# NVlabs/FoundationPose

Hardware: NVIDIA H100
Metric: pose-hypotheses/sec at 640x480 RGB-D, 252 hyp, 5 refine iters (higher is better)
Workload: dtype f16

## Files before the change

foundationpose_b200/csrc/fp_gemm.cu:

```cuda
#include "fp_gemm.cuh"

#include <stdarg.h>
#include <stdlib.h>
#include <string.h>

#include <mutex>
#include <vector>

#include "fp_common.cuh"
#include "fp_wgmma.cuh"

namespace fp {

static std::atomic<unsigned long long> g_launch_count{0};
static thread_local bool t_capturing = false;
void note_launches(int n) {
  if (!t_capturing) g_launch_count.fetch_add((unsigned long long)n, std::memory_order_relaxed);
}
unsigned long long launch_count() { return g_launch_count.load(std::memory_order_relaxed); }
void set_capturing(bool on) { t_capturing = on; }

std::atomic<bool> g_prof_on{false};
static std::mutex g_prof_mu;

struct ProfRec {
  cudaEvent_t e0, e1;
  double work;
  int kind;
};
static std::vector<ProfRec> g_prof_recs;

void prof_mark_begin(int kind, double work, cudaStream_t stream) {
  if (!g_prof_on) return;
  ProfRec r;
  r.kind = kind;
  r.work = work;
  cudaEventCreate(&r.e0);
  cudaEventCreate(&r.e1);
  cudaEventRecord(r.e0, stream);
  std::lock_guard<std::mutex> lk(g_prof_mu);
  g_prof_recs.push_back(r);
}
void prof_mark_end(cudaStream_t stream) {
  if (!g_prof_on) return;
  std::lock_guard<std::mutex> lk(g_prof_mu);
  if (g_prof_recs.empty()) return;
  cudaEventRecord(g_prof_recs.back().e1, stream);
}
int prof_collect(int kind, double* total_ms, double* total_work, int* launches) {
  FP_CUDA_OK(cudaDeviceSynchronize());
  std::lock_guard<std::mutex> lk(g_prof_mu);
  double ms = 0, work = 0;
  int n = 0;
  std::vector<ProfRec> keep;
  for (auto& r : g_prof_recs) {
    if (r.kind != kind) {
      keep.push_back(r);
      continue;
    }
    float t = 0.f;
    cudaEventElapsedTime(&t, r.e0, r.e1);
    ms += t;
    work += r.work;
    ++n;
    cudaEventDestroy(r.e0);
    cudaEventDestroy(r.e1);
  }
  g_prof_recs.swap(keep);
  *total_ms = ms;
  *total_work = work;
  *launches = n;
  return 0;
}

static thread_local char t_last_error[1024] = "";
void set_last_error(const char* fmt, ...) {
  va_list ap;
  va_start(ap, fmt);
  vsnprintf(t_last_error, sizeof(t_last_error), fmt, ap);
  va_end(ap);
}
const char* get_last_error() { return t_last_error; }

static thread_local int t_pdl_skip = 0;
void pdl_skip_next() { t_pdl_skip = 1; }

bool pdl_enabled() {
  if (t_pdl_skip) {
    t_pdl_skip = 0;
    return false;
  }
  static int on = -1;
  if (on < 0) {
    const char* e = getenv("FPOSE_PDL");
    on = (e && e[0] == '0') ? 0 : 1;
  }
  return on != 0;
}

struct GemmParams {
  int lg_bw, lg_bh;
  int bw, bh, bn;
  int tiles_w, tiles_h, tiles_n, n_tiles_n, total_tiles;
  int num_kb, chunks_per_tap;
  int dim_w, dim_h, dim_n;
  short tap_off[9][5];
  int Ho, Wo, n_img, Cout;
  const float* bias;
  int has_res;
  int odim_h, odim_n;
  int out_split;
  const float* post_add;
  int relu;
  double alg_flops;
};

constexpr int kBlockM = 128;
constexpr int kBlockK = 64;
constexpr int kABytes = kBlockM * kBlockK * 2;
constexpr int kTileThreads = 384;
constexpr int kSlabBytes = kBlockM * 64 * 2;
constexpr int kSmemOptIn = 232448;

constexpr int kWideSlabs = 2;
constexpr int kWideProducerRegs = 40;
constexpr int kWideConsumerRegs = 232;
template <int BN>
struct TileCfg {
  static constexpr int kBBytes = BN * kBlockK * 2;
  static constexpr int kStageBytes = kABytes + kBBytes;
  static constexpr int kBatches = BN / 64;
  static constexpr bool kAlternate = BN > 128;
  static constexpr int kSlabs = kAlternate ? kWideSlabs : kBatches;
  static constexpr int kStagingBytes = kSlabs * kSlabBytes;
  static constexpr int kRing = kSmemOptIn - kStagingBytes - 1024  - 256 ;
  static constexpr int kStages = (kRing / kStageBytes) > 8 ? 8 : (kRing / kStageBytes);
  static constexpr int kSmemBytes = kStages * kStageBytes + kStagingBytes + 1024 + 256;
  static_assert(kSmemBytes <= kSmemOptIn, "tile configuration exceeds the 227 KB opt-in shared memory");
  static_assert((2 * kStages + kSlabs) * 8 <= 256, "the mbarriers must fit their 256 bytes");
  static_assert(kBatches % kSlabs == 0, "every slab must take the same number of batches per tile");
};

template <int BN>
__global__ void __launch_bounds__(kTileThreads, 1)
    gemm_tile_kernel(const __grid_constant__ CUtensorMap map_a, const __grid_constant__ CUtensorMap map_b,
                     const __grid_constant__ CUtensorMap map_out, const __grid_constant__ CUtensorMap map_res,
                     const __grid_constant__ GemmParams p) {
  using Cfg = TileCfg<BN>;
  constexpr int S = Cfg::kStages;
  constexpr int NSLAB = Cfg::kSlabs;
  constexpr int NB = Cfg::kBatches;
  constexpr bool kAlt = Cfg::kAlternate;
  extern __shared__ uint8_t smem_raw[];
  uint8_t* smem = smem_raw + ((1024u - (smem_u32(smem_raw) & 1023u)) & 1023u);
  uint8_t* staging = smem + S * Cfg::kStageBytes;
  uint64_t* bars = reinterpret_cast<uint64_t*>(staging + Cfg::kStagingBytes);
  uint64_t* full = bars;
  uint64_t* empty = bars + S;
  uint64_t* res_full = bars + 2 * S;

  const int m_tiles = p.tiles_w * p.tiles_h * p.tiles_n;
  const int total = m_tiles * p.n_tiles_n;

  if (threadIdx.x == 0) {
    tma_prefetch_desc(&map_a);
    tma_prefetch_desc(&map_b);
    tma_prefetch_desc(&map_out);
    if (p.has_res) tma_prefetch_desc(&map_res);
    for (int s = 0; s < S; ++s) {
      mbar_init(&full[s], 1);
      mbar_init(&empty[s], 256);
    }
    for (int s = 0; s < (kAlt ? NSLAB : 1); ++s) mbar_init(&res_full[s], 1);
    mbar_fence_init();
  }
  __syncthreads();
  pdl_trigger();
  pdl_wait();

  auto decode = [&](int t, int& n_tile, int& tw, int& th, int& tn) {
    n_tile = t % p.n_tiles_n;
    const int m_tile = t / p.n_tiles_n;
    tw = m_tile % p.tiles_w;
    th = (m_tile / p.tiles_w) % p.tiles_h;
    tn = m_tile / (p.tiles_w * p.tiles_h);
  };

  if (threadIdx.x < 128) {
    if constexpr (BN > 128) regs_release<kWideProducerRegs>();
    if (threadIdx.x == 0) {
      int stage = 0, phase = 0;
      for (int t = blockIdx.x; t < total; t += gridDim.x) {
        int n_tile, tw, th, tn;
        decode(t, n_tile, tw, th, tn);
        int base[5] = {0, 0, 0, 0, 0};
        base[p.dim_w] += tw * p.bw;
        if (p.dim_h >= 0) base[p.dim_h] += th * p.bh;
        if (p.dim_n >= 0) base[p.dim_n] += tn * p.bn;
        int tap = 0, chunk = 0;
        for (int kb = 0; kb < p.num_kb; ++kb) {
          mbar_wait(&empty[stage], phase ^ 1);
          uint8_t* sa = smem + stage * Cfg::kStageBytes;
          mbar_expect_tx(&full[stage], Cfg::kStageBytes);
          tma_load_5d(&map_a, &full[stage], sa, base[0] + p.tap_off[tap][0] + chunk * kBlockK, base[1] + p.tap_off[tap][1],
                      base[2] + p.tap_off[tap][2], base[3] + p.tap_off[tap][3], base[4] + p.tap_off[tap][4]);
          tma_load_2d(&map_b, &full[stage], sa + kABytes, kb * kBlockK, n_tile * BN);
          if (++chunk == p.chunks_per_tap) {
            chunk = 0;
            ++tap;
          }
          if (++stage == S) {
            stage = 0;
            phase ^= 1;
          }
        }
      }
    }
    return;
  }

  if constexpr (BN > 128) regs_acquire<kWideConsumerRegs>();
  const int ct = threadIdx.x - 128;
  const int cw = ct >> 7;
  const int lane = threadIdx.x & 31;
  const int r0 = 64 * cw + 16 * ((ct >> 5) & 3) + (lane >> 2);
  const int cq = 2 * (lane & 3);
  const bool leader = (ct == 0);
  float acc[BN / 2];
#pragma unroll
  for (int i = 0; i < BN / 2; ++i) acc[i] = 0.f;
  int stage = 0, phase = 0, it = 0;
  for (int t = blockIdx.x; t < total; t += gridDim.x, ++it) {
    int n_tile, tw, th, tn;
    decode(t, n_tile, tw, th, tn);
    const int n0 = tn * p.bn;
    int n_o0 = n0, coff = 0;
    if (p.out_split > 0) {
      n_o0 = n0 % p.out_split;
      coff = (n0 / p.out_split) * p.Cout;
    }
    int oc[5] = {0, 0, 0, 0, 0}, rc[5] = {0, 0, 0, 0, 0};
    oc[1] = rc[1] = tw * p.bw;
    if (p.odim_h >= 0) oc[p.odim_h] = rc[p.odim_h] = th * p.bh;
    if (p.odim_n >= 0) {
      oc[p.odim_n] = n_o0;
      rc[p.odim_n] = n0;
    }
    if (leader) asm volatile("cp.async.bulk.wait_group.read 0;" ::: "memory");
    asm volatile("bar.sync 1, 256;" ::: "memory");
    if (leader && p.has_res) {
      for (int s = 0; s < NSLAB; ++s) {
        uint64_t* rb = &res_full[kAlt ? s : 0];
        if (kAlt || s == 0) mbar_expect_tx(rb, kAlt ? kSlabBytes : NSLAB * kSlabBytes);
        tma_load_5d(&map_res, rb, staging + s * kSlabBytes, n_tile * BN + s * 64, rc[1], rc[2], rc[3], rc[4]);
      }
    }

    int prev = -1;
    for (int kb = 0; kb < p.num_kb; ++kb) {
      mbar_wait(&full[stage], phase);
      const uint32_t sa = smem_u32(smem + stage * Cfg::kStageBytes);
      const uint64_t da = gmma_desc_sw128(sa + (uint32_t)cw * 8192u);
      const uint64_t db = gmma_desc_sw128(sa + kABytes);
      wgmma_fence();
#pragma unroll
      for (int k = 0; k < kBlockK / 16; ++k)
        Wgmma<BN>::ss(acc, da + (uint64_t)(2 * k), db + (uint64_t)(2 * k), (kb > 0 || k > 0) ? 1u : 0u);
      wgmma_commit();
      if (prev >= 0) {
        wgmma_wait<1>();
        mbar_arrive(&empty[prev]);
      }
      prev = stage;
      if (++stage == S) {
        stage = 0;
        phase ^= 1;
      }
    }
    const float* bias = p.bias + n_tile * BN;
    const float* pap[2] = {nullptr, nullptr};
    if (p.post_add) {
#pragma unroll
      for (int h = 0; h < 2; ++h) {
        const int row = r0 + 8 * h;
        const int jj = row & (p.bw - 1), ii = (row >> p.lg_bw) & (p.bh - 1);
        const int i = th * p.bh + ii, j = min(tw * p.bw + jj, p.Wo - 1);
        pap[h] = p.post_add + (size_t)(i * p.Wo + j) * p.Cout + n_tile * BN;
      }
    }
    float2 pe[8][2];
    auto load_pe = [&](int b) {
#pragma unroll
      for (int jl = 0; jl < 8; ++jl)
#pragma unroll
        for (int h = 0; h < 2; ++h) pe[jl][h] = __ldg(reinterpret_cast<const float2*>(pap[h] + 64 * b + 8 * jl + cq));
    };
    if (p.post_add) load_pe(0);
    wgmma_wait<0>();
    fence_regs(acc);
    if (prev >= 0) mbar_arrive(&empty[prev]);

#pragma unroll
    for (int b = 0; b < NB; ++b) {
      const int s = kAlt ? (b & 1) : b;
      uint8_t* slab = staging + s * kSlabBytes;
      if (kAlt && p.has_res && b > 0 && b + 1 < NB) {
        if (leader) {
          asm volatile("cp.async.bulk.wait_group.read 0;" ::: "memory");
          uint64_t* rb = &res_full[(b + 1) & 1];
          mbar_expect_tx(rb, kSlabBytes);
          tma_load_5d(&map_res, rb, staging + ((b + 1) & 1) * kSlabBytes, n_tile * BN + (b + 1) * 64, rc[1], rc[2],
                      rc[3], rc[4]);
        }
      }
      if (p.has_res && (kAlt || b == 0))
        mbar_wait(&res_full[kAlt ? s : 0], (uint32_t)((it * (NB / NSLAB) + b / NSLAB) & 1));
#pragma unroll
      for (int jh = 0; jh < 8; jh += 4) {
        float2 bb[4];
        __half2 rv[4][2];
#pragma unroll
        for (int jl = 0; jl < 4; ++jl) {
          bb[jl] = __ldg(reinterpret_cast<const float2*>(bias + 64 * b + 8 * (jh + jl) + cq));
          if (p.has_res) {
#pragma unroll
            for (int h = 0; h < 2; ++h) {
              const int row = r0 + 8 * h;
              rv[jl][h] = *reinterpret_cast<const __half2*>(slab + row * 128 + (((uint32_t)(jh + jl) ^ (uint32_t)(row & 7)) << 4) + cq * 2);
            }
          }
        }
#pragma unroll
        for (int jl = 0; jl < 4; ++jl) {
          const int j = 8 * b + jh + jl;
#pragma unroll
          for (int h = 0; h < 2; ++h) {
            const int row = r0 + 8 * h;
            uint32_t* cell = reinterpret_cast<uint32_t*>(slab + row * 128 + (((uint32_t)(jh + jl) ^ (uint32_t)(row & 7)) << 4) + cq * 2);
            float a0 = acc[4 * j + 2 * h] + bb[jl].x, a1 = acc[4 * j + 2 * h + 1] + bb[jl].y;
            if (p.has_res) {
              const float2 r = __half22float2(rv[jl][h]);
              a0 += r.x;
              a1 += r.y;
            }
            if (p.relu) {
              a0 = fmaxf(a0, 0.f);
              a1 = fmaxf(a1, 0.f);
            }
            if (p.post_add) {
              a0 += pe[jh + jl][h].x;
              a1 += pe[jh + jl][h].y;
            }
            *cell = pack_half2(a0, a1);
          }
        }
      }
      if (p.post_add && b + 1 < NB) load_pe(b + 1);
      if (kAlt || b == NB - 1) {
        asm volatile("fence.proxy.async.shared::cta;" ::: "memory");
        if (kAlt && leader) asm volatile("cp.async.bulk.wait_group.read 0;" ::: "memory");
        asm volatile("bar.sync 1, 256;" ::: "memory");
        if (leader) {
          for (int q = kAlt ? s : 0; q < (kAlt ? s + 1 : NSLAB); ++q)
            tma_store_5d(&map_out, staging + q * kSlabBytes, coff + n_tile * BN + (kAlt ? 64 * b : 64 * q), oc[1],
                         oc[2], oc[3], oc[4]);
          asm volatile("cp.async.bulk.commit_group;" ::: "memory");
        }
      }
    }
  }
  if (leader) asm volatile("cp.async.bulk.wait_group 0;" ::: "memory");
}

static int g_num_sms = 0;

typedef CUresult (*EncodeTiledFn)(CUtensorMap*, CUtensorMapDataType, cuuint32_t, void*, const cuuint64_t*,
                                  const cuuint64_t*, const cuuint32_t*, const cuuint32_t*,
                                  CUtensorMapInterleave, CUtensorMapSwizzle, CUtensorMapL2promotion,
                                  CUtensorMapFloatOOBfill);

static EncodeTiledFn get_encode_fn() {
  static EncodeTiledFn fn = nullptr;
  static std::once_flag once;
  std::call_once(once, [] {
    void* p = nullptr;
    cudaDriverEntryPointQueryResult qres;
    if (cudaGetDriverEntryPoint("cuTensorMapEncodeTiled", &p, cudaEnableDefault, &qres) == cudaSuccess &&
        qres == cudaDriverEntryPointSuccess)
      fn = reinterpret_cast<EncodeTiledFn>(p);
  });
  return fn;
}

static int encode_map(CUtensorMap* map, const void* base, int rank, const uint64_t* dims,
                      const uint64_t* strides_bytes , const uint32_t* box, bool swizzle128 = true) {
  EncodeTiledFn fn = get_encode_fn();
  FP_REQUIRE(fn != nullptr, "cuTensorMapEncodeTiled entry point not available (no CUDA driver?)");
  cuuint64_t gdim[5];
  cuuint64_t gstr[4];
  cuuint32_t bdim[5];
  cuuint32_t estr[5];
  for (int i = 0; i < rank; ++i) {
    gdim[i] = dims[i];
    bdim[i] = box[i];
    estr[i] = 1;
  }
  for (int i = 0; i < rank - 1; ++i) gstr[i] = strides_bytes[i];
  CUresult r = fn(map, CU_TENSOR_MAP_DATA_TYPE_FLOAT16, (cuuint32_t)rank, const_cast<void*>(base), gdim, gstr,
                  bdim, estr, CU_TENSOR_MAP_INTERLEAVE_NONE, swizzle128 ? CU_TENSOR_MAP_SWIZZLE_128B : CU_TENSOR_MAP_SWIZZLE_NONE,
                  CU_TENSOR_MAP_L2_PROMOTION_L2_256B, CU_TENSOR_MAP_FLOAT_OOB_FILL_NONE);
  FP_REQUIRE(r == CUDA_SUCCESS,
             "cuTensorMapEncodeTiled failed (%d): rank %d dims [%llu %llu %llu %llu %llu] box [%u %u %u %u %u]",
             (int)r, rank, (unsigned long long)dims[0], (unsigned long long)(rank > 1 ? dims[1] : 0),
             (unsigned long long)(rank > 2 ? dims[2] : 0), (unsigned long long)(rank > 3 ? dims[3] : 0),
             (unsigned long long)(rank > 4 ? dims[4] : 0), box[0], rank > 1 ? box[1] : 0, rank > 2 ? box[2] : 0,
             rank > 3 ? box[3] : 0, rank > 4 ? box[4] : 0);
  return 0;
}

int encode_map_f16(CUtensorMap* map, const void* base, int rank, const uint64_t* dims, const uint64_t* strides_bytes,
                   const uint32_t* box) {
  return encode_map(map, base, rank, dims, strides_bytes, box);
}
int encode_map_f16_linear(CUtensorMap* map, const void* base, int rank, const uint64_t* dims,
                          const uint64_t* strides_bytes, const uint32_t* box) {
  return encode_map(map, base, rank, dims, strides_bytes, box, false);
}
int num_sms() {
  if (g_num_sms == 0) {
    int dev = 0;
    if (cudaGetDevice(&dev) != cudaSuccess) return 0;
    if (cudaDeviceGetAttribute(&g_num_sms, cudaDevAttrMultiProcessorCount, dev) != cudaSuccess) return 0;
  }
  return g_num_sms;
}

static int ilog2(int v) {
  int l = 0;
  while ((1 << l) < v) ++l;
  return l;
}

template <int BN>
static int launch_bn(const CUtensorMap& ma, const CUtensorMap& mb, const CUtensorMap& mo, const CUtensorMap& mr,
                     const GemmParams& p, cudaStream_t stream) {
  using Cfg = TileCfg<BN>;
  static std::atomic<unsigned long long> attr_mask{0};
  if (!device_bit_test(attr_mask)) {
    FP_CUDA_OK(cudaFuncSetAttribute(gemm_tile_kernel<BN>, cudaFuncAttributeMaxDynamicSharedMemorySize, Cfg::kSmemBytes));
    device_bit_set(attr_mask);
  }
  const int sms = num_sms();
  FP_REQUIRE(sms > 0, "no CUDA device");
  const int grid = p.total_tiles < sms ? p.total_tiles : sms;
  prof_mark_begin(0, p.alg_flops, stream);
  FP_CUDA_OK(launch_pdl(gemm_tile_kernel<BN>, dim3(grid), dim3(kTileThreads), Cfg::kSmemBytes, stream, 1, ma, mb, mo, mr, p));
  prof_mark_end(stream);
  note_launches(1);
  FP_CUDA_OK(cudaGetLastError());
  return 0;
}

int stem_conv_launch(const GemmLayer& L, cudaStream_t stream);

static int gemm_layer_plan(const GemmLayer& L, cudaStream_t stream, int* tile_n) {
  if (L.kind == LK_CONV7_S2) {
    if (tile_n) {
      *tile_n = 64;
      return 0;
    }
    return stem_conv_launch(L, stream);
  }
  GemmParams p;
  memset(&p, 0, sizeof(p));
  CUtensorMap ma, mb;
  const uint64_t E = 2;
  int Ho, Wo, taps, ktot;
  int BN;
  uint64_t dims[5], str[4];
  uint32_t box[5];

  switch (L.kind) {
    case LK_LINEAR: {
      FP_REQUIRE(L.Cin % 64 == 0, "LINEAR: K=%d not a multiple of 64", L.Cin);
      Ho = 1;
      Wo = L.Win;
      taps = 1;
      p.chunks_per_tap = L.Cin / 64;
      p.bw = 128; p.bh = 1; p.bn = 1;
      p.dim_w = 1; p.dim_h = -1; p.dim_n = -1;
      dims[0] = L.Cin; dims[1] = L.Win; dims[2] = 1; dims[3] = 1; dims[4] = 1;
      str[0] = L.Cin * E; str[1] = str[0] * L.Win; str[2] = str[1]; str[3] = str[1];
      box[0] = 64; box[1] = 128; box[2] = 1; box[3] = 1; box[4] = 1;
      p.tiles_w = (L.Win + 127) / 128; p.tiles_h = 1; p.tiles_n = 1;
      break;
    }
    case LK_CONV3_S1: {
      FP_REQUIRE(L.Cin % 64 == 0, "CONV3_S1: Cin=%d not a multiple of 64", L.Cin);
      Ho = L.Hin; Wo = L.Win;
      taps = 9;
      p.chunks_per_tap = L.Cin / 64;
      if (Wo % 8 == 0 && Ho % 8 == 0) { p.bw = 8; p.bh = 8; p.bn = 2; }
      else if (Wo % 4 == 0 && Ho % 4 == 0) { p.bw = 4; p.bh = 4; p.bn = 8; }
      else FP_REQUIRE(false, "CONV3_S1: unsupported spatial size %dx%d", Ho, Wo);
      const uint64_t sw_ = (uint64_t)L.Cin * E, sh_ = sw_ * L.Win, sn_ = sh_ * L.Hin;
      p.dim_w = 1; p.dim_h = 2; p.dim_n = 3;
      dims[0] = L.Cin; dims[1] = L.Win; dims[2] = L.Hin; dims[3] = L.n_img; dims[4] = 1;
      str[0] = sw_; str[1] = sh_; str[2] = sn_; str[3] = sn_ * L.n_img;
      box[0] = 64; box[1] = p.bw; box[2] = p.bh; box[3] = p.bn; box[4] = 1;
      for (int r = 0; r < 3; ++r)
        for (int s = 0; s < 3; ++s) {
          p.tap_off[r * 3 + s][1] = (short)(s - 1);
          p.tap_off[r * 3 + s][2] = (short)(r - 1);
        }
      p.tiles_w = Wo / p.bw; p.tiles_h = Ho / p.bh; p.tiles_n = (L.n_img + p.bn - 1) / p.bn;
      break;
    }
    case LK_CONV3_S2: {
      FP_REQUIRE(L.Cin % 64 == 0, "CONV3_S2: Cin=%d not a multiple of 64", L.Cin);
      FP_REQUIRE(L.Hin % 2 == 0 && L.Win % 2 == 0, "CONV3_S2: odd input size");
      Ho = L.Hin / 2; Wo = L.Win / 2;
      taps = 9;
      p.chunks_per_tap = L.Cin / 64;
      if (Wo % 8 == 0 && Ho % 8 == 0) { p.bw = 8; p.bh = 8; p.bn = 2; }
      else if (Wo % 4 == 0 && Ho % 4 == 0) { p.bw = 4; p.bh = 4; p.bn = 8; }
      else FP_REQUIRE(false, "CONV3_S2: unsupported output size %dx%d", Ho, Wo);
      p.dim_w = 1; p.dim_h = 3; p.dim_n = 4;
      dims[0] = 2 * L.Cin; dims[1] = Wo; dims[2] = 2; dims[3] = Ho; dims[4] = L.n_img;
      str[0] = 2 * L.Cin * E; str[1] = (uint64_t)L.Win * L.Cin * E; str[2] = 2 * str[1];
      str[3] = (uint64_t)L.Hin * L.Win * L.Cin * E;
      box[0] = 64; box[1] = p.bw; box[2] = 1; box[3] = p.bh; box[4] = p.bn;
      for (int r = 0; r < 3; ++r)
        for (int s = 0; s < 3; ++s) {
          const int t = r * 3 + s;
          p.tap_off[t][0] = (short)((s == 1 ? 0 : 1) * L.Cin);
          p.tap_off[t][1] = (short)(s == 0 ? -1 : 0);
          p.tap_off[t][2] = (short)(r == 1 ? 0 : 1);
          p.tap_off[t][3] = (short)(r == 0 ? -1 : 0);
        }
      p.tiles_w = Wo / p.bw; p.tiles_h = Ho / p.bh; p.tiles_n = (L.n_img + p.bn - 1) / p.bn;
      break;
    }
    default:
      FP_REQUIRE(false, "unknown layer kind %d", L.kind);
  }
  ktot = taps * L.Cin;
  p.num_kb = ktot / 64;
  p.lg_bw = ilog2(p.bw);
  p.lg_bh = ilog2(p.bh);

  constexpr int kWideMinWaves = 8;
  constexpr int kWideMinKBlocks = 16;
  const int m_tiles = p.tiles_w * p.tiles_h * p.tiles_n;
  if (L.Cout % 256 == 0 && p.num_kb >= kWideMinKBlocks) {
    const int sms = num_sms();
    FP_REQUIRE(sms > 0, "no CUDA device");
    BN = (long long)m_tiles * (L.Cout / 256) >= (long long)kWideMinWaves * sms ? 256 : 128;
  } else if (L.Cout % 128 == 0) BN = 128;
  else if (L.Cout % 64 == 0) BN = 64;
  else FP_REQUIRE(false, "Cout=%d must be a multiple of 64", L.Cout);
  p.n_tiles_n = L.Cout / BN;
  p.total_tiles = p.tiles_w * p.tiles_h * p.tiles_n * p.n_tiles_n;
  p.Ho = Ho; p.Wo = Wo; p.n_img = L.n_img; p.Cout = L.Cout;
  p.bias = L.bias;
  p.has_res = L.res != nullptr;
  p.out_split = L.out_split;
  p.post_add = L.post_add;
  p.relu = L.relu;
  {
    const double k_real = (double)taps * L.Cin;
    p.alg_flops = 2.0 * (double)L.n_img * Ho * Wo * L.Cout * k_real;
  }
  FP_REQUIRE(L.out_ld % 8 == 0 && (!L.res || L.res_ld % 8 == 0), "out_ld / res_ld must be multiples of 8");
  FP_REQUIRE(L.out_split == 0 || L.out_split % p.bn == 0,
             "out_split=%d must be a multiple of the tile's image count %d (pad the A/B batch boundary)", L.out_split,
             p.bn);
  if (tile_n) {
    *tile_n = BN;
    return 0;
  }
  if (p.total_tiles == 0) return 0;

  int rc = encode_map(&ma, L.in, 5, dims, str, box);
  if (rc) return rc;
  uint64_t wd[2] = {(uint64_t)ktot, (uint64_t)L.Cout};
  uint64_t ws[1] = {(uint64_t)ktot * E};
  uint32_t wb[2] = {64, (uint32_t)BN};
  rc = encode_map(&mb, L.w, 2, wd, ws, wb);
  if (rc) return rc;
  CUtensorMap mo, mr;
  {
    uint64_t od[5], os[4];
    uint32_t ob[5];
    const bool lin = (L.kind == LK_LINEAR);
    const int n_out = L.out_split > 0 ? (L.n_img - L.out_split) : L.n_img;
    FP_REQUIRE(n_out > 0, "out_split=%d leaves no output images (n_img=%d)", L.out_split, L.n_img);
    auto fill = [&](int ld, int nimg) {
      const uint64_t sw_ = (uint64_t)ld * E, sh_ = sw_ * Wo, sn_ = sh_ * Ho;
      od[0] = (uint64_t)ld;
      ob[0] = 64;
      od[4] = 1;
      ob[4] = 1;
      if (lin) {
        od[1] = (uint64_t)Wo; od[2] = 1; od[3] = 1;
        os[0] = sw_; os[1] = sh_; os[2] = sh_; os[3] = sh_;
        ob[1] = (uint32_t)p.bw; ob[2] = 1; ob[3] = 1;
      } else {
        od[1] = (uint64_t)Wo; od[2] = (uint64_t)Ho; od[3] = (uint64_t)nimg;
        os[0] = sw_; os[1] = sh_; os[2] = sn_; os[3] = sn_ * nimg;
        ob[1] = (uint32_t)p.bw; ob[2] = (uint32_t)p.bh; ob[3] = (uint32_t)p.bn;
      }
    };
    p.odim_h = lin ? -1 : 2;
    p.odim_n = lin ? -1 : 3;
    fill(L.out_ld, n_out);
    rc = encode_map(&mo, L.out, 5, od, os, ob);
    if (rc) return rc;
    if (L.res) {
      fill(L.res_ld, L.n_img);
      rc = encode_map(&mr, L.res, 5, od, os, ob);
      if (rc) return rc;
    } else {
      mr = mo;
    }
  }
  if (BN == 256) return launch_bn<256>(ma, mb, mo, mr, p, stream);
  return BN == 128 ? launch_bn<128>(ma, mb, mo, mr, p, stream) : launch_bn<64>(ma, mb, mo, mr, p, stream);
}

int gemm_layer_launch(const GemmLayer& L, cudaStream_t stream) { return gemm_layer_plan(L, stream, nullptr); }

int gemm_layer_tile_n(const GemmLayer& L, int* tile_n) { return gemm_layer_plan(L, nullptr, tile_n); }

}
```

Before: 3611.

## Overlap next tile's first k-blocks with epilogue using double accumulators

```diff
diff --git a/foundationpose_b200/csrc/fp_gemm.cu b/foundationpose_b200/csrc/fp_gemm.cu
--- a/foundationpose_b200/csrc/fp_gemm.cu
+++ b/foundationpose_b200/csrc/fp_gemm.cu
@@ -123,8 +123,10 @@
 constexpr int kSmemOptIn = 232448;
 
 constexpr int kWideSlabs = 2;
-constexpr int kWideProducerRegs = 40;
-constexpr int kWideConsumerRegs = 232;
+constexpr int kProducerRegs = 40;
+constexpr int kConsumerRegs = 232;
+constexpr int kOverlapHead = 3;
+constexpr int kOverlapMaxKBlocks = 8;
 template <int BN>
 struct TileCfg {
   static constexpr int kBBytes = BN * kBlockK * 2;
@@ -139,7 +141,53 @@
   static_assert(kSmemBytes <= kSmemOptIn, "tile configuration exceeds the 227 KB opt-in shared memory");
   static_assert((2 * kStages + kSlabs) * 8 <= 256, "the mbarriers must fit their 256 bytes");
   static_assert(kBatches % kSlabs == 0, "every slab must take the same number of batches per tile");
+  static_assert(kAlternate || kOverlapHead < kStages, "the overlapped k-blocks need free ring stages");
 };
+
+template <int BN>
+__device__ __forceinline__ void convert_batch(const float (&acc)[BN / 2], int b, uint8_t* slab, const float* bias,
+                                              const float2 (&pe)[8][2], const GemmParams& p, int r0, int cq) {
+#pragma unroll
+  for (int jh = 0; jh < 8; jh += 4) {
+    float2 bb[4];
+    __half2 rv[4][2];
+#pragma unroll
+    for (int jl = 0; jl < 4; ++jl) {
+      bb[jl] = __ldg(reinterpret_cast<const float2*>(bias + 64 * b + 8 * (jh + jl) + cq));
+      if (p.has_res) {
+#pragma unroll
+        for (int h = 0; h < 2; ++h) {
+          const int row = r0 + 8 * h;
+          rv[jl][h] = *reinterpret_cast<const __half2*>(slab + row * 128 + (((uint32_t)(jh + jl) ^ (uint32_t)(row & 7)) << 4) + cq * 2);
+        }
+      }
+    }
+#pragma unroll
+    for (int jl = 0; jl < 4; ++jl) {
+      const int j = 8 * b + jh + jl;
+#pragma unroll
+      for (int h = 0; h < 2; ++h) {
+        const int row = r0 + 8 * h;
+        uint32_t* cell = reinterpret_cast<uint32_t*>(slab + row * 128 + (((uint32_t)(jh + jl) ^ (uint32_t)(row & 7)) << 4) + cq * 2);
+        float a0 = acc[4 * j + 2 * h] + bb[jl].x, a1 = acc[4 * j + 2 * h + 1] + bb[jl].y;
+        if (p.has_res) {
+          const float2 r = __half22float2(rv[jl][h]);
+          a0 += r.x;
+          a1 += r.y;
+        }
+        if (p.relu) {
+          a0 = fmaxf(a0, 0.f);
+          a1 = fmaxf(a1, 0.f);
+        }
+        if (p.post_add) {
+          a0 += pe[jh + jl][h].x;
+          a1 += pe[jh + jl][h].y;
+        }
+        *cell = pack_half2(a0, a1);
+      }
+    }
+  }
+}
 
 template <int BN>
 __global__ void __launch_bounds__(kTileThreads, 1)
@@ -187,7 +235,7 @@
   };
 
   if (threadIdx.x < 128) {
-    if constexpr (BN > 128) regs_release<kWideProducerRegs>();
+    regs_release<kProducerRegs>();
     if (threadIdx.x == 0) {
       int stage = 0, phase = 0;
       for (int t = blockIdx.x; t < total; t += gridDim.x) {
@@ -219,45 +267,53 @@
     return;
   }
 
-  if constexpr (BN > 128) regs_acquire<kWideConsumerRegs>();
+  regs_acquire<kConsumerRegs>();
   const int ct = threadIdx.x - 128;
   const int cw = ct >> 7;
   const int lane = threadIdx.x & 31;
   const int r0 = 64 * cw + 16 * ((ct >> 5) & 3) + (lane >> 2);
   const int cq = 2 * (lane & 3);
   const bool leader = (ct == 0);
-  float acc[BN / 2];
-#pragma unroll
-  for (int i = 0; i < BN / 2; ++i) acc[i] = 0.f;
-  int stage = 0, phase = 0, it = 0;
-  for (int t = blockIdx.x; t < total; t += gridDim.x, ++it) {
-    int n_tile, tw, th, tn;
-    decode(t, n_tile, tw, th, tn);
-    const int n0 = tn * p.bn;
-    int n_o0 = n0, coff = 0;
-    if (p.out_split > 0) {
-      n_o0 = n0 % p.out_split;
-      coff = (n0 / p.out_split) * p.Cout;
-    }
-    int oc[5] = {0, 0, 0, 0, 0}, rc[5] = {0, 0, 0, 0, 0};
-    oc[1] = rc[1] = tw * p.bw;
-    if (p.odim_h >= 0) oc[p.odim_h] = rc[p.odim_h] = th * p.bh;
-    if (p.odim_n >= 0) {
-      oc[p.odim_n] = n_o0;
-      rc[p.odim_n] = n0;
-    }
-    if (leader) asm volatile("cp.async.bulk.wait_group.read 0;" ::: "memory");
-    asm volatile("bar.sync 1, 256;" ::: "memory");
-    if (leader && p.has_res) {
-      for (int s = 0; s < NSLAB; ++s) {
-        uint64_t* rb = &res_full[kAlt ? s : 0];
-        if (kAlt || s == 0) mbar_expect_tx(rb, kAlt ? kSlabBytes : NSLAB * kSlabBytes);
-        tma_load_5d(&map_res, rb, staging + s * kSlabBytes, n_tile * BN + s * 64, rc[1], rc[2], rc[3], rc[4]);
-      }
-    }
-
-    int prev = -1;
-    for (int kb = 0; kb < p.num_kb; ++kb) {
+  if constexpr (!kAlt) {
+    int stage = 0, phase = 0;
+
+    auto tile_coords = [&](int t, int& n_tile, int& tw, int& th, int& coff, int (&oc)[5], int (&rc)[5]) {
+      int tn;
+      decode(t, n_tile, tw, th, tn);
+      const int n0 = tn * p.bn;
+      int n_o0 = n0;
+      coff = 0;
+      if (p.out_split > 0) {
+        n_o0 = n0 % p.out_split;
+        coff = (n0 / p.out_split) * p.Cout;
+      }
+#pragma unroll
+      for (int d = 0; d < 5; ++d) oc[d] = rc[d] = 0;
+      oc[1] = rc[1] = tw * p.bw;
+      if (p.odim_h >= 0) oc[p.odim_h] = rc[p.odim_h] = th * p.bh;
+      if (p.odim_n >= 0) {
+        oc[p.odim_n] = n_o0;
+        rc[p.odim_n] = n0;
+      }
+    };
+    const float* pap[2] = {nullptr, nullptr};
+    float2 pe[8][2];
+    auto pe_rows = [&](int n_tile, int tw, int th) {
+#pragma unroll
+      for (int h = 0; h < 2; ++h) {
+        const int row = r0 + 8 * h;
+        const int jj = row & (p.bw - 1), ii = (row >> p.lg_bw) & (p.bh - 1);
+        const int i = th * p.bh + ii, j = min(tw * p.bw + jj, p.Wo - 1);
+        pap[h] = p.post_add + (size_t)(i * p.Wo + j) * p.Cout + n_tile * BN;
+      }
+    };
+    auto load_pe = [&](int b) {
+#pragma unroll
+      for (int jl = 0; jl < 8; ++jl)
+#pragma unroll
+        for (int h = 0; h < 2; ++h) pe[jl][h] = __ldg(reinterpret_cast<const float2*>(pap[h] + 64 * b + 8 * jl + cq));
+    };
+    auto mma_kblock = [&](float (&acc)[BN / 2], int kb) {
       mbar_wait(&full[stage], phase);
       const uint32_t sa = smem_u32(smem + stage * Cfg::kStageBytes);
       const uint64_t da = gmma_desc_sw128(sa + (uint32_t)cw * 8192u);
@@ -267,104 +323,233 @@
       for (int k = 0; k < kBlockK / 16; ++k)
         Wgmma<BN>::ss(acc, da + (uint64_t)(2 * k), db + (uint64_t)(2 * k), (kb > 0 || k > 0) ? 1u : 0u);
       wgmma_commit();
-      if (prev >= 0) {
-        wgmma_wait<1>();
-        mbar_arrive(&empty[prev]);
-      }
-      prev = stage;
       if (++stage == S) {
         stage = 0;
         phase ^= 1;
       }
-    }
-    const float* bias = p.bias + n_tile * BN;
-    const float* pap[2] = {nullptr, nullptr};
-    if (p.post_add) {
-#pragma unroll
-      for (int h = 0; h < 2; ++h) {
-        const int row = r0 + 8 * h;
-        const int jj = row & (p.bw - 1), ii = (row >> p.lg_bw) & (p.bh - 1);
-        const int i = th * p.bh + ii, j = min(tw * p.bw + jj, p.Wo - 1);
-        pap[h] = p.post_add + (size_t)(i * p.Wo + j) * p.Cout + n_tile * BN;
-      }
-    }
-    float2 pe[8][2];
-    auto load_pe = [&](int b) {
-#pragma unroll
-      for (int jl = 0; jl < 8; ++jl)
-#pragma unroll
-        for (int h = 0; h < 2; ++h) pe[jl][h] = __ldg(reinterpret_cast<const float2*>(pap[h] + 64 * b + 8 * jl + cq));
     };
-    if (p.post_add) load_pe(0);
-    wgmma_wait<0>();
-    fence_regs(acc);
-    if (prev >= 0) mbar_arrive(&empty[prev]);
-
-#pragma unroll
-    for (int b = 0; b < NB; ++b) {
-      const int s = kAlt ? (b & 1) : b;
-      uint8_t* slab = staging + s * kSlabBytes;
-      if (kAlt && p.has_res && b > 0 && b + 1 < NB) {
-        if (leader) {
-          asm volatile("cp.async.bulk.wait_group.read 0;" ::: "memory");
-          uint64_t* rb = &res_full[(b + 1) & 1];
-          mbar_expect_tx(rb, kSlabBytes);
-          tma_load_5d(&map_res, rb, staging + ((b + 1) & 1) * kSlabBytes, n_tile * BN + (b + 1) * 64, rc[1], rc[2],
-                      rc[3], rc[4]);
-        }
-      }
-      if (p.has_res && (kAlt || b == 0))
-        mbar_wait(&res_full[kAlt ? s : 0], (uint32_t)((it * (NB / NSLAB) + b / NSLAB) & 1));
-#pragma unroll
-      for (int jh = 0; jh < 8; jh += 4) {
-        float2 bb[4];
-        __half2 rv[4][2];
-#pragma unroll
-        for (int jl = 0; jl < 4; ++jl) {
-          bb[jl] = __ldg(reinterpret_cast<const float2*>(bias + 64 * b + 8 * (jh + jl) + cq));
-          if (p.has_res) {
+
+    float acc0[BN / 2], acc1[BN / 2];
+    const int head = min(kOverlapHead, p.num_kb);
+    int rel = 0, held = 0;
+    auto release_to = [&](int keep) {
+      for (; held > keep; --held) {
+        mbar_arrive(&empty[rel]);
+        if (++rel == S) rel = 0;
+      }
+    };
+    int issued = 0;
+    auto run_tile = [&](float (&acc)[BN / 2], float (&nxt)[BN / 2], int t, int it) {
+      int n_tile, tw, th, coff, oc[5], rc[5];
+      tile_coords(t, n_tile, tw, th, coff, oc, rc);
+      if (leader && p.has_res) {
+        asm volatile("cp.async.bulk.wait_group.read 0;" ::: "memory");
+        mbar_expect_tx(&res_full[0], NSLAB * kSlabBytes);
+        for (int s = 0; s < NSLAB; ++s)
+          tma_load_5d(&map_res, &res_full[0], staging + s * kSlabBytes, n_tile * BN + s * 64, rc[1], rc[2], rc[3], rc[4]);
+      }
+      for (int kb = issued; kb < p.num_kb; ++kb) {
+        mma_kblock(acc, kb);
+        ++held;
+        wgmma_wait<1>();
+        release_to(1);
+      }
+      const float* bias = p.bias + n_tile * BN;
+      if (p.post_add) {
+        pe_rows(n_tile, tw, th);
+        load_pe(0);
+      }
+      const bool has_next = t + (int)gridDim.x < total;
+      const bool overlap = has_next && head == kOverlapHead && p.num_kb <= kOverlapMaxKBlocks;
+      issued = 0;
+      if (overlap) {
+        wgmma_wait<0>();
+        release_to(0);
+#pragma unroll
+        for (int kb = 0; kb < kOverlapHead; ++kb) mma_kblock(nxt, kb);
+        issued = kOverlapHead;
+        held += kOverlapHead;
+      } else {
+        if (has_next)
+          for (; issued < head; ++issued) mma_kblock(nxt, issued);
+        held += issued;
+        wgmma_wait<0>();
+        release_to(0);
+      }
+      fence_regs(acc);
+      if (p.has_res) {
+        mbar_wait(&res_full[0], (uint32_t)(it & 1));
+      } else {
+        if (leader) asm volatile("cp.async.bulk.wait_group.read 0;" ::: "memory");
+        asm volatile("bar.sync 1, 256;" ::: "memory");
+      }
+#pragma unroll
+      for (int b = 0; b < NB; ++b) {
+        convert_batch<BN>(acc, b, staging + b * kSlabBytes, bias, pe, p, r0, cq);
+        if (b + 1 < NB) {
+          if (p.post_add) load_pe(b + 1);
+          if (overlap && issued < p.num_kb) {
+            mma_kblock(nxt, issued++);
+            ++held;
+            wgmma_wait<kOverlapHead>();
+            release_to(kOverlapHead);
+          }
+        }
+      }
+      asm volatile("fence.proxy.async.shared::cta;" ::: "memory");
+      asm volatile("bar.sync 1, 256;" ::: "memory");
+      if (leader) {
+        for (int q = 0; q < NSLAB; ++q)
+          tma_store_5d(&map_out, staging + q * kSlabBytes, coff + n_tile * BN + 64 * q, oc[1], oc[2], oc[3], oc[4]);
+        asm volatile("cp.async.bulk.commit_group;" ::: "memory");
+      }
+    };
+    for (int t = blockIdx.x, it = 0; t < total; t += gridDim.x, ++it) {
+      run_tile(acc0, acc1, t, it);
+      if ((t += gridDim.x) >= total) break;
+      run_tile(acc1, acc0, t, ++it);
+    }
+  } else {
+    float acc[BN / 2];
+#pragma unroll
+    for (int i = 0; i < BN / 2; ++i) acc[i] = 0.f;
+    int stage = 0, phase = 0, it = 0;
+    for (int t = blockIdx.x; t < total; t += gridDim.x, ++it) {
+      int n_tile, tw, th, tn;
+      decode(t, n_tile, tw, th, tn);
+      const int n0 = tn * p.bn;
+      int n_o0 = n0, coff = 0;
+      if (p.out_split > 0) {
+        n_o0 = n0 % p.out_split;
+        coff = (n0 / p.out_split) * p.Cout;
+      }
+      int oc[5] = {0, 0, 0, 0, 0}, rc[5] = {0, 0, 0, 0, 0};
+      oc[1] = rc[1] = tw * p.bw;
+      if (p.odim_h >= 0) oc[p.odim_h] = rc[p.odim_h] = th * p.bh;
+      if (p.odim_n >= 0) {
+        oc[p.odim_n] = n_o0;
+        rc[p.odim_n] = n0;
+      }
+      if (leader) asm volatile("cp.async.bulk.wait_group.read 0;" ::: "memory");
+      asm volatile("bar.sync 1, 256;" ::: "memory");
+      if (leader && p.has_res) {
+        for (int s = 0; s < NSLAB; ++s) {
+          uint64_t* rb = &res_full[kAlt ? s : 0];
+          if (kAlt || s == 0) mbar_expect_tx(rb, kAlt ? kSlabBytes : NSLAB * kSlabBytes);
+          tma_load_5d(&map_res, rb, staging + s * kSlabBytes, n_tile * BN + s * 64, rc[1], rc[2], rc[3], rc[4]);
+        }
+      }
+
+      int prev = -1;
+      for (int kb = 0; kb < p.num_kb; ++kb) {
+        mbar_wait(&full[stage], phase);
+        const uint32_t sa = smem_u32(smem + stage * Cfg::kStageBytes);
+        const uint64_t da = gmma_desc_sw128(sa + (uint32_t)cw * 8192u);
+        const uint64_t db = gmma_desc_sw128(sa + kABytes);
+        wgmma_fence();
+#pragma unroll
+        for (int k = 0; k < kBlockK / 16; ++k)
+          Wgmma<BN>::ss(acc, da + (uint64_t)(2 * k), db + (uint64_t)(2 * k), (kb > 0 || k > 0) ? 1u : 0u);
+        wgmma_commit();
+        if (prev >= 0) {
+          wgmma_wait<1>();
+          mbar_arrive(&empty[prev]);
+        }
+        prev = stage;
+        if (++stage == S) {
+          stage = 0;
+          phase ^= 1;
+        }
+      }
+      const float* bias = p.bias + n_tile * BN;
+      const float* pap[2] = {nullptr, nullptr};
+      if (p.post_add) {
+#pragma unroll
+        for (int h = 0; h < 2; ++h) {
+          const int row = r0 + 8 * h;
+          const int jj = row & (p.bw - 1), ii = (row >> p.lg_bw) & (p.bh - 1);
+          const int i = th * p.bh + ii, j = min(tw * p.bw + jj, p.Wo - 1);
+          pap[h] = p.post_add + (size_t)(i * p.Wo + j) * p.Cout + n_tile * BN;
+        }
+      }
+      float2 pe[8][2];
+      auto load_pe = [&](int b) {
+#pragma unroll
+        for (int jl = 0; jl < 8; ++jl)
+#pragma unroll
+          for (int h = 0; h < 2; ++h) pe[jl][h] = __ldg(reinterpret_cast<const float2*>(pap[h] + 64 * b + 8 * jl + cq));
+      };
+      if (p.post_add) load_pe(0);
+      wgmma_wait<0>();
+      fence_regs(acc);
+      if (prev >= 0) mbar_arrive(&empty[prev]);
+
+#pragma unroll
+      for (int b = 0; b < NB; ++b) {
+        const int s = kAlt ? (b & 1) : b;
+        uint8_t* slab = staging + s * kSlabBytes;
+        if (kAlt && p.has_res && b > 0 && b + 1 < NB) {
+          if (leader) {
+            asm volatile("cp.async.bulk.wait_group.read 0;" ::: "memory");
+            uint64_t* rb = &res_full[(b + 1) & 1];
+            mbar_expect_tx(rb, kSlabBytes);
+            tma_load_5d(&map_res, rb, staging + ((b + 1) & 1) * kSlabBytes, n_tile * BN + (b + 1) * 64, rc[1], rc[2],
+                        rc[3], rc[4]);
+          }
+        }
+        if (p.has_res && (kAlt || b == 0))
+          mbar_wait(&res_full[kAlt ? s : 0], (uint32_t)((it * (NB / NSLAB) + b / NSLAB) & 1));
+#pragma unroll
+        for (int jh = 0; jh < 8; jh += 4) {
+          float2 bb[4];
+          __half2 rv[4][2];
+#pragma unroll
+          for (int jl = 0; jl < 4; ++jl) {
+            bb[jl] = __ldg(reinterpret_cast<const float2*>(bias + 64 * b + 8 * (jh + jl) + cq));
+            if (p.has_res) {
+#pragma unroll
+              for (int h = 0; h < 2; ++h) {
+                const int row = r0 + 8 * h;
+                rv[jl][h] = *reinterpret_cast<const __half2*>(slab + row * 128 + (((uint32_t)(jh + jl) ^ (uint32_t)(row & 7)) << 4) + cq * 2);
+              }
+            }
+          }
+#pragma unroll
+          for (int jl = 0; jl < 4; ++jl) {
+            const int j = 8 * b + jh + jl;
 #pragma unroll
             for (int h = 0; h < 2; ++h) {
               const int row = r0 + 8 * h;
-              rv[jl][h] = *reinterpret_cast<const __half2*>(slab + row * 128 + (((uint32_t)(jh + jl) ^ (uint32_t)(row & 7)) << 4) + cq * 2);
+              uint32_t* cell = reinterpret_cast<uint32_t*>(slab + row * 128 + (((uint32_t)(jh + jl) ^ (uint32_t)(row & 7)) << 4) + cq * 2);
+              float a0 = acc[4 * j + 2 * h] + bb[jl].x, a1 = acc[4 * j + 2 * h + 1] + bb[jl].y;
+              if (p.has_res) {
+                const float2 r = __half22float2(rv[jl][h]);
+                a0 += r.x;
+                a1 += r.y;
+              }
+              if (p.relu) {
+                a0 = fmaxf(a0, 0.f);
+                a1 = fmaxf(a1, 0.f);
+              }
+              if (p.post_add) {
+                a0 += pe[jh + jl][h].x;
+                a1 += pe[jh + jl][h].y;
+              }
+              *cell = pack_half2(a0, a1);
             }
           }
         }
-#pragma unroll
-        for (int jl = 0; jl < 4; ++jl) {
-          const int j = 8 * b + jh + jl;
-#pragma unroll
-          for (int h = 0; h < 2; ++h) {
-            const int row = r0 + 8 * h;
-            uint32_t* cell = reinterpret_cast<uint32_t*>(slab + row * 128 + (((uint32_t)(jh + jl) ^ (uint32_t)(row & 7)) << 4) + cq * 2);
-            float a0 = acc[4 * j + 2 * h] + bb[jl].x, a1 = acc[4 * j + 2 * h + 1] + bb[jl].y;
-            if (p.has_res) {
-              const float2 r = __half22float2(rv[jl][h]);
-              a0 += r.x;
-              a1 += r.y;
-            }
-            if (p.relu) {
-              a0 = fmaxf(a0, 0.f);
-              a1 = fmaxf(a1, 0.f);
-            }
-            if (p.post_add) {
-              a0 += pe[jh + jl][h].x;
-              a1 += pe[jh + jl][h].y;
-            }
-            *cell = pack_half2(a0, a1);
+        if (p.post_add && b + 1 < NB) load_pe(b + 1);
+        if (kAlt || b == NB - 1) {
+          asm volatile("fence.proxy.async.shared::cta;" ::: "memory");
+          if (kAlt && leader) asm volatile("cp.async.bulk.wait_group.read 0;" ::: "memory");
+          asm volatile("bar.sync 1, 256;" ::: "memory");
+          if (leader) {
+            for (int q = kAlt ? s : 0; q < (kAlt ? s + 1 : NSLAB); ++q)
+              tma_store_5d(&map_out, staging + q * kSlabBytes, coff + n_tile * BN + (kAlt ? 64 * b : 64 * q), oc[1],
+                           oc[2], oc[3], oc[4]);
+            asm volatile("cp.async.bulk.commit_group;" ::: "memory");
           }
-        }
-      }
-      if (p.post_add && b + 1 < NB) load_pe(b + 1);
-      if (kAlt || b == NB - 1) {
-        asm volatile("fence.proxy.async.shared::cta;" ::: "memory");
-        if (kAlt && leader) asm volatile("cp.async.bulk.wait_group.read 0;" ::: "memory");
-        asm volatile("bar.sync 1, 256;" ::: "memory");
-        if (leader) {
-          for (int q = kAlt ? s : 0; q < (kAlt ? s + 1 : NSLAB); ++q)
-            tma_store_5d(&map_out, staging + q * kSlabBytes, coff + n_tile * BN + (kAlt ? 64 * b : 64 * q), oc[1],
-                         oc[2], oc[3], oc[4]);
-          asm volatile("cp.async.bulk.commit_group;" ::: "memory");
         }
       }
     }
```

Measured after the change: 3611, median of 6. Within noise of the previous version (-0.0%).
